# jyjblrd/Low-Cost-Mocap

Hardware: AMD Instinct MI355X
Metric: triangulated 3D markers/sec at 8 cams x 16 markers (higher is better)
Workload: dtype f64

## Files before the change

low-cost-mocap_amd/csrc/frame_bb.hip:

```cpp
#include "mocap_device.hpp"
#include "kernels.hpp"
#include <cstdlib>
#include "frame_common.hpp"
#include "bb_fold.hpp"

namespace mocap {

constexpr int kBBThreads = 256;
constexpr int kBBWaves = kBBThreads / 64;
constexpr int kBBRecs = kBBThreads + 64;
constexpr int bb_cw(int C) { return C <= 8 ? 1 : 2; }
constexpr uint32_t bb_rec_bytes(int CW) { return 24u + 8u * (uint32_t)CW; }
constexpr bool bb_group_rows(int CT, int ML, int RL) { return CT > 0 && ML > 0 && RL > 0 && CT * ML < 0xFF && (ML & (ML - 1)) == 0; }

constexpr int bb_wg_per_cu(int RL) { return RL == 48 ? 5 : 4; }
constexpr size_t kBBCacheEntry = 4;
constexpr int kBBLdsSlack = 1024;
struct BBLayout {
  size_t bxy, bxy_nx, cnt_nx, bt, rbound, seedkey, slot_key, claimw, recs, rpk, scr, scr_bytes, goff, gcnt, outslot, boff, bnb, seedgh, slot_g, cnt,
      misc, bpl, nh, hits, act, root_blob, root_cam, nact, bnl, bv, pkbase, seen, bcache, total;
  int ncache;
  __host__ __device__ static size_t al(size_t x, size_t a) { return (x + a - 1) / a * a; }
  __host__ __device__ BBLayout(int C, int M, int R, int CW, int wg_per_cu) {
    size_t o = 0;
    auto take = [&](size_t bytes, size_t a) {
      o = al(o, a);
      const size_t at = o;
      o += bytes;
      return at;
    };
    bxy = take(sizeof(float2) * (size_t)C * M, 16);
    bxy_nx = take(sizeof(float2) * (size_t)C * M, 16);
    cnt_nx = take(4 * (size_t)C, 4);
    bt = take(sizeof(double) * 10 * ((size_t)C * M + 1), 16);
    rbound = take(8 * (size_t)R, 8);
    claimw = take(8 * (size_t)C, 8);
    pkbase = take(8 * (size_t)CW * R, 8);
    scr = seedkey = take(8 * (size_t)R, 8);
    slot_key = take(8 * (size_t)kBBWaves * R, 8);
    recs = take(8 * (size_t)kBBRecs, 8);
    rpk = take(8 * (size_t)kBBRecs * CW, 8);
    seedgh = take(4 * (size_t)R, 4);
    slot_g = take(4 * (size_t)kBBWaves * R, 4);
    scr_bytes = o - scr;
    goff = take(4 * (size_t)(R + 1), 4);
    gcnt = take(4 * (size_t)R, 4);
    outslot = take(4 * (size_t)R, 4);
    boff = take(4 * (size_t)(R + 1), 4);
    bnb = take(4 * (size_t)R, 4);
    cnt = take(4 * (size_t)C, 4);
    misc = take(4 * 16, 4);
    bpl = take(2 * (size_t)R, 2);
    seen = take(2 * (size_t)R, 2);
    nh = take((size_t)R * C, 1);
    hits = take((size_t)R * C * M, 1);
    act = take((size_t)R * C, 1);
    root_blob = take((size_t)R, 1);
    root_cam = take((size_t)R, 1);
    nact = take((size_t)R, 1);
    bnl = take((size_t)R, 1);
    bv = take((size_t)R, 1);
    bcache = take(0, 4);
    ncache = 0;
    const size_t per_entry = kBBCacheEntry;
    for (int per_cu = wg_per_cu; per_cu >= 1; per_cu--) {
      const size_t lim = ((size_t)160 * 1024 / per_cu - kBBLdsSlack) / 256 * 256;
      if (lim >= o + per_entry * 64) {
        const size_t n = (lim - o) / per_entry;
        ncache = (int)(n > 1024 ? 1024 : n);
        break;
      }
    }
    o += per_entry * (size_t)ncache;
    total = al(o, 16);
  }
};

static int bb_fixed_slots(int C, int M, int R) {
  const char* e = getenv("MOCAP_BB_FIXED_LAYOUT");
  if (e && e[0] == '0') return 0;
  if (C == 8 && M == 16 && R <= 48) return 48;
  if (C == 8 && M == 16 && R <= 64) return 64;
  return 0;
}
static int frame_bb_root_slots(int C, int M, int R) {
  const int f = bb_fixed_slots(C, M, R);
  return f ? f : R;
}
size_t frame_bb_lds_bytes(int C, int M, int R) { return BBLayout(C, M, frame_bb_root_slots(C, M, R), bb_cw(C), bb_wg_per_cu(bb_fixed_slots(C, M, R))).total; }
static size_t frame_bb_lds_bytes_min(int C, int M, int R) {
  const BBLayout L(C, M, frame_bb_root_slots(C, M, R), bb_cw(C), bb_wg_per_cu(bb_fixed_slots(C, M, R)));
  return L.total - kBBCacheEntry * (size_t)L.ncache;
}
bool frame_bb_fits(int C, int M, int R) {
  return C >= 2 && C <= 16 && M >= 1 && M <= 64 && R >= 1 && R <= 255 && frame_bb_lds_bytes_min(C, M, R) <= (size_t)128 * 1024;
}

template <int CW, uint32_t NONE = 0xFFu>
struct Packed {
  unsigned long long w[CW];
  __device__ __forceinline__ void clear() {
#pragma unroll
    for (int k = 0; k < CW; k++) w[k] = NONE * 0x0101010101010101ull;
  }
  __device__ __forceinline__ void set(int c, uint32_t idx) {
    if (CW == 1)
      w[0] ^= (unsigned long long)(idx ^ NONE) << (8 * c);
    else
      w[c >> 3] ^= (unsigned long long)(idx ^ NONE) << (8 * (c & 7));
  }
  __device__ __forceinline__ uint32_t get(int c) const {
    return CW == 1 ? (uint32_t)(w[0] >> (8 * c)) & 0xFFu : (uint32_t)(w[c >> 3] >> (8 * (c & 7))) & 0xFFu;
  }
};

template <int CT, bool PERK = false>
struct BBCamTables {
  const double* base;
  static constexpr int C = CT;
  static constexpr int kPq = PERK ? 12 * CT * CT : 12 * CT;
  __device__ __forceinline__ ctab_t pq(size_t off) const { return as_ctab(base + off); }
  __device__ __forceinline__ ctab_t rt(size_t off) const { return as_ctab(base + kPq + off); }
  __device__ __forceinline__ ctab_t k4(size_t off) const { return as_ctab(base + kPq + 12 * CT + off); }
  __device__ __forceinline__ const double* f() const { return base + kPq + 16 * CT; }
};
template <bool PERK>
struct BBCamTables<0, PERK> {
  const double* base;
  int C;
  __device__ __forceinline__ ctab_t pq(size_t off) const { return as_ctab(base + off); }
  __device__ __forceinline__ ctab_t rt(size_t off) const { return as_ctab(base + (PERK ? 12 * C * C : 12 * C) + off); }
  __device__ __forceinline__ ctab_t k4(size_t off) const { return as_ctab(base + (PERK ? 12 * C * C + 12 * C : 24 * C) + off); }
  __device__ __forceinline__ const double* f() const { return base + (PERK ? 12 * C * C + 16 * C : 28 * C); }
};

enum { kPrioEval = 0, kPrioSeed = 1, kPrioPhase = 2, kPrioSerial = 3 };
template <int P>
__device__ __forceinline__ void bb_prio() {
  __builtin_amdgcn_s_setprio(P);
}

template <bool F32R, int CW, int CT, int ML, int RL, bool PERK = false>
struct BBState {
  static constexpr int T = kBBThreads, W = kBBWaves;
  static constexpr bool ROWS = bb_group_rows(CT, ML, RL);
  static constexpr uint32_t kNone = ROWS ? (uint32_t)(CT * ML) : 0xFFu;
  typedef Packed<CW, kNone> Pk;
  static constexpr bool PLIST = CT > 0 && ML > 0 && RL > 0 && ML < 32 && CT * ML <= 256 && (ML & (ML - 1)) == 0;
  __device__ __forceinline__ uint32_t gbyte(int c, uint32_t k) const { return ROWS ? (uint32_t)c * (uint32_t)ML + k : k; }
  __device__ __forceinline__ size_t grow(int c, uint32_t b) const { return ROWS ? (size_t)b : (size_t)c * M + b; }
  const FrameArgs& p;
  BBCamTables<CT, PERK> cv;
  const int C_, M, R, RS;
  int tid, lane, wave;
  __device__ __forceinline__ void fresh_tid() {
    int t = tid;
    asm volatile("" : "+v"(t));
    tid = t;
    lane = t & 63;
    wave = t >> 6;
  }
  __device__ __forceinline__ int cn() const { return CT > 0 ? CT : C_; }
  enum { PC_OTHER = 0, PC_PAIRS0, PC_PAIRS1, PC_B1_TABLE, PC_ROW_COPY, PC_PHASE_C, PC_SEED_PASS, PC_SEED_PUSH, PC_EVAL, PC_TEST, PC_PHASE_E, PC_COUNT };
#ifdef MOCAP_BB_PHASE_CLOCKS
  uint32_t pc_last = 0, pc_sum[PC_COUNT] = {};
  template <int PH>
  __device__ __forceinline__ void pc_mark() {
    if (__builtin_amdgcn_readfirstlane((int)threadIdx.x >> 6) == 0) {
      const uint32_t now = (uint32_t)__builtin_readcyclecounter();
      pc_sum[PH] += now - pc_last;
      pc_last = now;
    }
  }
  __device__ __forceinline__ void pc_start() { pc_last = (uint32_t)__builtin_readcyclecounter(); }
  __device__ __forceinline__ void pc_flush() const {
    if (threadIdx.x == 0 && !p.n_frames_dev)
      for (int k = 0; k < PC_COUNT; k++) atomicAdd(&p.status[p.n_frames + k], (int)(pc_sum[k] >> 8));
  }
#else
  template <int PH>
  __device__ __forceinline__ void pc_mark() {}
  __device__ __forceinline__ void pc_start() {}
  __device__ __forceinline__ void pc_flush() const {}
#endif
  double* bt;
  float2 *bxy, *bxy_nx;
  int32_t* cnt_nx;
  unsigned long long *rbound, *seedkey, *slot_key, *claimw, *rpk;
  struct BRec { uint32_t gh, rs; };
  BRec* recs;
  uint32_t *goff, *gcnt, *boff, *bnb, *seedgh, *slot_g;
  int32_t *outslot, *cnt, *misc;
  uint16_t* bpl;
  uint8_t *nh, *hits, *act, *root_blob, *root_cam, *nact, *bnl, *bv;
  float* bcache;
  unsigned long long* pkbase;
  uint16_t* seen;
  int ncache;
  unsigned char* scr;
  size_t scr_bytes;
  static constexpr unsigned long long kInfBits = 0x7ff0000000000000ull;

  __device__ BBState(const FrameArgs& p_, unsigned char* smem)
      : p(p_), C_(p_.cv.C), M(ML > 0 ? ML : p_.M), R(p_.K_max), RS(RL > 0 ? RL : p_.K_max), tid(threadIdx.x), lane(threadIdx.x & 63), wave(threadIdx.x >> 6) {
    const int C = cn();
    {
      const unsigned long long ta = (unsigned long long)(uintptr_t)p_.cv.Pq;
      uint32_t tlo = (uint32_t)__builtin_amdgcn_readfirstlane((int)(uint32_t)ta);
      uint32_t thi = (uint32_t)__builtin_amdgcn_readfirstlane((int)(uint32_t)(ta >> 32));
      asm volatile("" : "+s"(tlo), "+s"(thi));
      cv.base = (const double*)(uintptr_t)(((unsigned long long)thi << 32) | tlo);
      if constexpr (CT == 0) cv.C = C;
    }
    const BBLayout L(C, M, RS, CW, bb_wg_per_cu(RL));
    bt = (double*)(smem + L.bt);
    bxy = (float2*)(smem + L.bxy);
    bxy_nx = (float2*)(smem + L.bxy_nx);
    cnt_nx = (int32_t*)(smem + L.cnt_nx);
    rbound = (unsigned long long*)(smem + L.rbound);
    seedkey = (unsigned long long*)(smem + L.seedkey);
    slot_key = (unsigned long long*)(smem + L.slot_key);
    claimw = (unsigned long long*)(smem + L.claimw);
    recs = (BRec*)(smem + L.recs);
    rpk = (unsigned long long*)(smem + L.rpk);
    goff = (uint32_t*)(smem + L.goff);
    gcnt = (uint32_t*)(smem + L.gcnt);
    outslot = (int32_t*)(smem + L.outslot);
    boff = (uint32_t*)(smem + L.boff);
    bnb = (uint32_t*)(smem + L.bnb);
    seedgh = (uint32_t*)(smem + L.seedgh);
    slot_g = (uint32_t*)(smem + L.slot_g);
    cnt = (int32_t*)(smem + L.cnt);
    misc = (int32_t*)(smem + L.misc);
    bpl = (uint16_t*)(smem + L.bpl);
    nh = (uint8_t*)(smem + L.nh);
    hits = (uint8_t*)(smem + L.hits);
    act = (uint8_t*)(smem + L.act);
    root_blob = (uint8_t*)(smem + L.root_blob);
    root_cam = (uint8_t*)(smem + L.root_cam);
    nact = (uint8_t*)(smem + L.nact);
    bnl = (uint8_t*)(smem + L.bnl);
    bv = (uint8_t*)(smem + L.bv);
    scr = smem + L.scr;
    scr_bytes = L.scr_bytes;
    bcache = (float*)(smem + L.bcache);
    pkbase = (unsigned long long*)(smem + L.pkbase);
    seen = (uint16_t*)(smem + L.seen);
    ncache = L.ncache;
  }

  struct Line { double a, b, c, den, rden; };
  __device__ __forceinline__ Line epiline(int r, int i) const { return epiline_of(root_cam[r], root_blob[r], i); }
  __device__ __forceinline__ Line epiline_of(int rc, int rb, int i) const {
    const int C = cn();
    const double* Fm = cv.f() + 9 * ((size_t)rc * C + i);
    const float2 rp = bxy[(size_t)rc * M + rb];
    const double x = (double)rp.x, y = (double)rp.y;
    double a = Fm[0] * x + Fm[1] * y + Fm[2];
    double b = Fm[3] * x + Fm[4] * y + Fm[5];
    double c = Fm[6] * x + Fm[7] * y + Fm[8];
    double nu = a * a + b * b;
    nu = nu != 0.0 ? 1.0 / sqrt(nu) : 1.0;
    a *= nu;
    b *= nu;
    c *= nu;
    if (F32R) {
      a = (double)(float)a;
      b = (double)(float)b;
      c = (double)(float)c;
    }
    Line L;
    L.a = a;
    L.b = b;
    L.c = c;
    L.den = sqrt(a * a + b * b);
    L.rden = recip_refined(L.den);
    return L;
  }

  template <bool CHAIN>
  __device__ __forceinline__ unsigned long long match_pairs(const Line& mine, int pair_r, int pair_i, int n_pairs, int gs_shift,
                                                            int cam = 0, int Mi_chain = 0) {
    const int C = cn();
    const int GS = 1 << gs_shift, PPS = 64 >> gs_shift;
    const int k = lane & (GS - 1), q = lane >> gs_shift;
    const int gl0 = lane & ~(GS - 1);
    const unsigned long long gall = gs_shift == 6 ? ~0ull : ((1ull << GS) - 1ull);
    unsigned long long claims = 0ull;
    for (int s0 = 0; s0 < n_pairs; s0 += PPS) {
      const int src = s0 + q;
      const bool has = src < n_pairs;
      const int sl = has ? src : 0;
      const double la = __shfl(mine.a, sl), lb = __shfl(mine.b, sl), lc = __shfl(mine.c, sl);
      const double lden = __shfl(mine.den, sl), lrden = __shfl(mine.rden, sl);
      const int r = __shfl(pair_r, sl);
      const int i = CHAIN ? cam : __shfl(pair_i, sl);
      const int Mi = has ? (CHAIN ? Mi_chain : cnt[i]) : 0;
      const bool valid = k < Mi;
      float2 pt = make_float2(0.f, 0.f);
      double d = 0.0;
      bool hit = false;
      if (valid) {
        pt = bxy[(size_t)i * M + k];
        const double num = fabs(la * (double)pt.x + lb * (double)pt.y + lc);
        d = div_by(num, lden, lrden);
        hit = d < p.gate_px;
      }
      const unsigned long long wm = __ballot(hit);
      const unsigned long long gm = (wm >> gl0) & gall;
      int rank = 0;
      const unsigned int dlo = (unsigned int)__double_as_longlong(d), dhi = (unsigned int)(__double_as_longlong(d) >> 32);
      for (unsigned long long mm = wm; mm;) {
        const int j = __ffsll((long long)mm) - 1;
        mm &= mm - 1;
        const double dj = __longlong_as_double(((long long)__builtin_amdgcn_readlane((int)dhi, j) << 32) |
                                               (unsigned int)__builtin_amdgcn_readlane((int)dlo, j));
        const bool mine_grp = (j & ~(GS - 1)) == gl0 && j != lane;
        rank += (hit && mine_grp && (dj < d || (dj == d && j < lane))) ? 1 : 0;
      }
      if (hit) hits[((size_t)r * C + i) * M + rank] = (uint8_t)gbyte(i, (uint32_t)k);
      const unsigned long long g0 = (__ballot(hit && rank == 0) >> gl0) & gall;
      bool same = false;
      if (valid && g0) {
        const float2 p0 = bxy[(size_t)i * M + (__ffsll((long long)g0) - 1)];
        same = pt.x == p0.x && pt.y == p0.y;
      }
      const unsigned long long cw = __ballot(same);
      if (CHAIN) {
        for (int sh = 0; sh < 64; sh += GS) claims |= (cw >> sh) & gall;
      }
      if (has && k == 0) {
        nh[(size_t)r * C + i] = (uint8_t)__popcll(gm);
        if (!CHAIN) {
          const unsigned long long cm = (cw >> gl0) & gall;
          if (cm) atomicOr(&claimw[i], cm);
        }
      }
    }
    return claims;
  }

  __device__ __forceinline__ void prefetch_lds(int64_t frame) const {
    const int C = cn();
    const float* src = p.blobs + (size_t)frame * C * M * 2;
    const int n_dw = C * M * 2;
    for (int base = wave * 64; base < n_dw; base += T)
      if (base + lane < n_dw)
        __builtin_amdgcn_global_load_lds((const __attribute__((address_space(1))) void*)(src + base + lane),
                                         (__attribute__((address_space(3))) void*)((float*)bxy_nx + base), 4, 0, 0);
    if (wave == 0 && lane < C)
      __builtin_amdgcn_global_load_lds((const __attribute__((address_space(1))) void*)(p.counts + (size_t)frame * C + lane),
                                       (__attribute__((address_space(3))) void*)cnt_nx, 4, 0, 0);
  }
  __device__ __forceinline__ void stage(int64_t frame) {
    fresh_tid();
    const int C = cn();
    float2* t = bxy;
    bxy = bxy_nx;
    bxy_nx = t;
    if (tid < C) {
      const int n = cnt_nx[tid];
      cnt[tid] = n < 0 ? 0 : (n > M ? M : n);
      claimw[tid] = 0ull;
    }
    if (tid == 0) {
      misc[MI_STATUS] = 0;
      misc[MI_OMAX] = 0;
    }
  }

  __device__ void match() {
    fresh_tid();
    const int C = cn();
    __syncthreads();
    int gs_shift = 0;
    while ((1 << gs_shift) < M) gs_shift++;
    const int n0 = cnt[0] < R ? cnt[0] : R;
    {
      for (int r = tid; r < n0; r += T) {
        root_cam[r] = 0;
        root_blob[r] = (uint8_t)r;
      }
      if (tid == 0 && cnt[0] > R) misc[MI_STATUS] |= MOCAP_ST_ROOT_OVERFLOW_;
    }
    __syncthreads();
    auto U_of = [&](int j) {
      const int n = cnt[j];
      return ~claimw[j] & (n >= 64 ? ~0ull : ((1ull << n) - 1ull));
    };
    int n_prov = 0, n_ppairs = 0;
    bool pre = false;
    uint8_t* nh_s = nullptr;
    uint8_t* hits_s = nullptr;
    unsigned long long* pclaim = (unsigned long long*)scr;
    uint8_t* plist = act;
    uint32_t* p_end = goff;
    {
      int Mmax = 0;
      for (int c = 1; c < C; c++) Mmax = cnt[c] > Mmax ? cnt[c] : Mmax;
#pragma nounroll
      for (int stage_ = 0; stage_ < 2; stage_++) {
        const int stage = __builtin_amdgcn_readfirstlane(stage_);
        int NP = n0 * (C - 1);
        if (stage == 1) {
          block_sync_lds();
          pc_mark<PC_PAIRS0>();
          if constexpr (PLIST) {
#pragma unroll
            for (int j = 1; j < CT; j++) {
              const uint32_t U = ~((const uint32_t*)claimw)[2 * j] & ((1u << cnt[j]) - 1u);
              if (lane < ML && ((U >> lane) & 1u)) plist[__builtin_amdgcn_mbcnt_lo(U, (uint32_t)n_prov)] = (uint8_t)(j * ML + lane);
              n_prov += __popc(U);
              n_ppairs += __popc(U) * (CT - 1 - j);
              if (lane == 0) p_end[j] = ((uint32_t)n_ppairs << 16) | (uint32_t)n_prov;
            }
            wave_lds_sync();
          } else
          for (int j = 1; j < C; j++) {
            const int np = __popcll(U_of(j));
            n_prov += np;
            n_ppairs += np * (C - 1 - j);
          }
          pre = n_prov <= 64 && (size_t)n_prov * C * (8 + 1 + (size_t)M) <= scr_bytes;
          if (!pre) break;
          nh_s = (uint8_t*)(pclaim + (size_t)n_prov * C);
          hits_s = nh_s + (size_t)n_prov * C;
          NP = n_ppairs;
        }
        for (int base = wave * 64; base < NP; base += W * 64) {
          const int pi = base + lane;
          const bool have = pi < NP;
          int r = 0, i = 1, Mi = 0;
          Line L = {0, 0, 0, 1, 1};
          if (have) {
            if (stage == 0) {
              r = pi / (C - 1);
              i = 1 + (pi - r * (C - 1));
              L = epiline(r, i);
            } else if constexpr (PLIST) {
              int j = 1;
              uint32_t before = 0;
              const uint32_t key = ((uint32_t)pi << 16) | 0xFFFFu;
              uint32_t pe[CT > 2 ? CT - 2 : 1];
#pragma unroll
              for (int jj = 1; jj <= CT - 2; jj++) pe[jj - 1] = p_end[jj];
#pragma unroll
              for (int jj = 1; jj <= CT - 2; jj++) {
                const bool ge = key >= pe[jj - 1];
                j += ge ? 1 : 0;
                before = ge ? pe[jj - 1] : before;
              }
              const uint32_t acc = before >> 16, pb = before & 0xFFFFu;
              uint32_t ord, off;
              divmod_tiny((uint32_t)pi - acc, (uint32_t)(CT - 1 - j), ord, off);
              r = (int)(pb + ord);
              const int k = plist[r] & (ML - 1);
              i = j + 1 + (int)off;
              L = epiline_of(j, k, i);
            } else {
              int j = 1, acc = 0, pb = 0, span = C - 2;
              unsigned long long U = 0ull;
              for (; j <= C - 2; j++) {
                span = C - 1 - j;
                U = U_of(j);
                const int nj = __popcll(U) * span;
                if (pi < acc + nj) break;
                acc += nj;
                pb += __popcll(U);
              }
              uint32_t ord, off;
              divmod_tiny((uint32_t)(pi - acc), (uint32_t)span, ord, off);
              for (uint32_t t = 0; t < ord; t++) U &= U - 1;
              const int k = __ffsll((long long)U) - 1;
              i = j + 1 + (int)off;
              r = pb + (int)ord;
              L = epiline_of(j, k, i);
            }
            Mi = cnt[i];
          }
          const float2* pts = bxy + (size_t)i * M;
          auto dist = [&](int k) {
            const float2 pt = pts[k];
            return div_by(fabs(L.a * (double)pt.x + L.b * (double)pt.y + L.c), L.den, L.rden);
          };
          unsigned long long hm = 0ull;
#pragma unroll 4
          for (int k = 0; k < Mmax; k++)
            if (k < Mi && dist(k) < p.gate_px) hm |= 1ull << k;
          uint8_t* nhp = stage == 0 ? nh : nh_s;
          uint8_t* hl = (stage == 0 ? hits : hits_s) + ((size_t)r * C + i) * M;
          if (have) nhp[(size_t)r * C + i] = (uint8_t)__popcll(hm);
          unsigned long long rem = hm, claim = 0ull;
          int pos = 0;
          float2 p0 = make_float2(0.f, 0.f);
          while (__ballot(rem != 0ull)) {
            if (rem) {
              double bd = __builtin_huge_val();
              int bk = 0;
              for (unsigned long long t = rem; t; t &= t - 1) {
                const int k = __ffsll((long long)t) - 1;
                const double d = dist(k);
                if (d < bd) {
                  bd = d;
                  bk = k;
                }
              }
              hl[pos] = (uint8_t)gbyte(i, (uint32_t)bk);
              if (pos == 0) {
                p0 = pts[bk];
                for (unsigned long long t = hm; t; t &= t - 1) {
                  const int k = __ffsll((long long)t) - 1;
                  const float2 q = pts[k];
                  if (q.x == p0.x && q.y == p0.y) claim |= 1ull << k;
                }
              }
              rem &= ~(1ull << bk);
              pos++;
            }
          }
          if (stage == 0) {
            if (claim) atomicOr(&claimw[i], claim);
          } else if (have) {
            pclaim[(size_t)r * C + i] = claim;
          }
        }
      }
    }
    const int NL = M * ((C - 1) * (C - 2) / 2);
    const bool spec = F32R && (size_t)NL * 20 + 8 <= scr_bytes;
    double* sp_den = (double*)scr;
    float* sp_abc = (float*)(sp_den + NL);
    auto sp_base = [&](int j) { return M * ((j - 1) * (C - 1) - (j - 1) * j / 2); };
    if (spec && !pre) {
      int tot = 0;
      for (int j = 1; j <= C - 2; j++) {
        const int n = cnt[j];
        const unsigned long long U = ~claimw[j] & (n >= 64 ? ~0ull : ((1ull << n) - 1ull));
        tot += __popcll(U) * (C - 1 - j);
      }
      for (int l = tid; l < tot; l += T) {
        int j = 1, acc = 0, span = C - 2;
        unsigned long long U = 0ull;
        for (; j <= C - 2; j++) {
          const int n = cnt[j];
          U = ~claimw[j] & (n >= 64 ? ~0ull : ((1ull << n) - 1ull));
          span = C - 1 - j;
          const int nj = __popcll(U) * span;
          if (l < acc + nj) break;
          acc += nj;
        }
        uint32_t ord, off;
        divmod_tiny((uint32_t)(l - acc), (uint32_t)span, ord, off);
        for (uint32_t t = 0; t < ord; t++) U &= U - 1;
        const int k = __ffsll((long long)U) - 1, i = j + 1 + (int)off;
        const int ll = sp_base(j) + k * span + (int)off;
        const Line L = epiline_of(j, k, i);
        sp_den[ll] = L.den;
        sp_abc[3 * ll + 0] = (float)L.a;
        sp_abc[3 * ll + 1] = (float)L.b;
        sp_abc[3 * ll + 2] = (float)L.c;
      }
    }
    __syncthreads();
    pc_mark<PC_PAIRS1>();
    fresh_tid();
    if (wave == 0) bb_prio<kPrioSerial>();
    if (wave == 0 && pre) {
      int jp = 0, kp = 0;
      if constexpr (PLIST) {
        if (lane < n_prov) {
          const int row = plist[lane];
          jp = row / ML;
          kp = row & (ML - 1);
        }
      } else
      if (lane < n_prov) {
        int acc = 0;
        unsigned long long U = 0ull;
        for (jp = 1; jp < C; jp++) {
          U = U_of(jp);
          const int np = __popcll(U);
          if (lane < acc + np) break;
          acc += np;
        }
        for (int t = 0; t < lane - acc; t++) U &= U - 1;
        kp = __ffsll((long long)U) - 1;
      }
      bool real = false;
      for (int i = 1; i < C; i++) {
        wave_lds_sync();
        if (lane < n_prov && jp == i) {
          real = !((claimw[i] >> kp) & 1ull);
          if (real)
            for (int c = i + 1; c < C; c++) {
              const unsigned long long m = pclaim[(size_t)lane * C + c];
              if (m) atomicOr(&claimw[c], m);
            }
        }
      }
      const unsigned long long rm = __ballot(real);
      const int rank = __popcll(rm & ((1ull << lane) - 1ull));
      int n_roots = n0 + __popcll(rm);
      if (real && n0 + rank < R) {
        root_cam[n0 + rank] = (uint8_t)jp;
        root_blob[n0 + rank] = (uint8_t)kp;
        bnl[rank] = (uint8_t)lane;
      }
      if (lane == 0) {
        if (n_roots > R) {
          misc[MI_STATUS] |= MOCAP_ST_ROOT_OVERFLOW_;
          n_roots = R;
        }
        misc[MI_NROOTS] = n_roots;
      }
    } else if (wave == 0) {
      const int cntL = lane < C ? cnt[lane] : 0;
      const unsigned long long clmL = lane < C ? claimw[lane] : 0ull;
      int nr_cam = 0, nr_blob = 0;
      int n_roots = n0;
      bool over = false;
      for (int i = 1; i < C; i++) {
        const int Mi = __builtin_amdgcn_readlane(cntL, i);
        unsigned long long claimed = ((unsigned long long)(unsigned int)__builtin_amdgcn_readlane((int)(clmL >> 32), i) << 32) |
                                     (unsigned int)__builtin_amdgcn_readlane((int)clmL, i);
        const int n_new = n_roots - n0;
        for (int base = 0; base < n_new; base += 64) {
          const int l = base + lane;
          const bool have = l < n_new;
          int j = nr_cam, k = nr_blob;
          if (base) {
            wave_lds_sync();
            j = have ? root_cam[n0 + l] : 0;
            k = have ? root_blob[n0 + l] : 0;
          }
          Line L = {0, 0, 0, 1, 1};
          if (have) {
            if (spec) {
              const int ll = sp_base(j) + k * (C - 1 - j) + (i - j - 1);
              L.a = (double)sp_abc[3 * ll + 0];
              L.b = (double)sp_abc[3 * ll + 1];
              L.c = (double)sp_abc[3 * ll + 2];
              L.den = sp_den[ll];
              L.rden = recip_refined(L.den);
            } else {
              L = epiline_of(j, k, i);
            }
          }
          claimed |= match_pairs<true>(L, n0 + l, i, (n_new - base < 64) ? n_new - base : 64, gs_shift, i, Mi);
        }
        const bool flag = lane < Mi && !((claimed >> lane) & 1ull);
        const unsigned long long mask = __ballot(flag);
        const int pos = __popcll(mask & ((1ull << lane) - 1ull));
        if (flag) {
          const int rr = n_roots + pos;
          if (rr < R) {
            root_cam[rr] = (uint8_t)i;
            root_blob[rr] = (uint8_t)lane;
          }
        }
        int slot = n_new;
        for (unsigned long long mm = mask; mm; slot++) {
          const int jb = __ffsll((long long)mm) - 1;
          mm &= mm - 1;
          if (lane == slot) {
            nr_cam = i;
            nr_blob = jb;
          }
        }
        n_roots += __popcll(mask);
        if (n_roots > R) {
          over = true;
          n_roots = R;
        }
      }
      if (lane == 0) {
        if (over) misc[MI_STATUS] |= MOCAP_ST_ROOT_OVERFLOW_;
        misc[MI_NROOTS] = n_roots;
      }
    } else {
      float om = 0.0f;
      for (int i = tid - 64; i < C * M; i += T - 64) {
        const int c = i / M, k = i - c * M;
        if (k < cnt[c]) {
          const float2 v = bxy[i];
          om = fmaxf(om, fmaxf(fabsf(v.x), fabsf(v.y)));
          double Bc[10];
          dlt_contribution(Bc, cv.pq(PERK ? 12 * (c * C + c) : 12 * c), (double)v.x, (double)v.y);
#pragma unroll
          for (int e = 0; e < 10; e++) bt[(size_t)i * 10 + e] = Bc[e];
        }
      }
      if (om > 0.0f) atomicMax(&misc[MI_OMAX], __float_as_int(om));
      if (tid == 64) {
        const int it = q_add(&p.q.counters[QC_NEXT_FRAME], 1);
        misc[MI_NEXT] = it < frame_count(p) ? it : -1;
      }
    }
    bb_prio<kPrioPhase>();
    __syncthreads();
    pc_mark<PC_B1_TABLE>();
    if (pre) {
      const int n_new = misc[MI_NROOTS] - n0;
      for (int idx = tid; idx < n_new * C; idx += T) {
        const int q = idx / C, c = idx - q * C;
        const int r = n0 + q, ps = bnl[q];
        if (c > (int)root_cam[r]) {
          const int n = nh_s[(size_t)ps * C + c];
          nh[(size_t)r * C + c] = (uint8_t)n;
          const uint8_t* src = hits_s + ((size_t)ps * C + c) * M;
          uint8_t* dst = hits + ((size_t)r * C + c) * M;
          for (int t = 0; t < n; t++) dst[t] = src[t];
        }
      }
      __syncthreads();
      pc_mark<PC_ROW_COPY>();
    }

    fresh_tid();
    const int nroots = misc[MI_NROOTS];
    for (int r = tid; r < nroots; r += T) {
      const int rc = root_cam[r];
      unsigned long long total = 1;
      int views = 1, na = 0;
      bool over = false;
      Pk pkb;
      pkb.clear();
      pkb.set(rc, gbyte(rc, root_blob[r]));
      uint32_t sm = 1u << rc;
      for (int c = rc + 1; c < C; c++) {
        const unsigned n = nh[(size_t)r * C + c];
        if (n > 1) act[(size_t)r * C + na++] = (uint8_t)c;
        if (n == 1) pkb.set(c, hits[((size_t)r * C + c) * M]);
        if (n) {
          sm |= 1u << c;
          views++;
          total *= n;
          if (total > (unsigned long long)p.G_cap) {
            over = true;
            total = 1;
          }
        }
      }
      if (over) atomicOr(&misc[MI_STATUS], MOCAP_ST_CAND_OVERFLOW_);
      nact[r] = (uint8_t)na;
      bv[r] = (uint8_t)views;
#pragma unroll
      for (int k = 0; k < CW; k++) pkbase[(size_t)r * CW + k] = pkb.w[k];
      if (PERK) seen[r] = (uint16_t)sm;
      rbound[r] = kInfBits;
      const uint32_t g = (views > 1 && !over) ? (uint32_t)total : 0u;
      gcnt[r] = g;
      {
        const uint8_t* a = act + (size_t)r * C;
        uint32_t pl = 1, nb = 1;
        int nl = 0;
        for (int k = 0; k < na; k++) nb *= nh[(size_t)r * C + a[k]];
        if (over) nb = 1;
        while (nl < na && (pl < (uint32_t)p.bb_pl_min || (pl < (uint32_t)p.bb_pl && nb > (uint32_t)p.bb_nb_max))) {
          const uint32_t n = nh[(size_t)r * C + a[nl++]];
          uint32_t dummy;
          pl *= n;
          divmod_small(nb, n, nb, dummy);
        }
        bpl[r] = (uint16_t)pl;
        bnl[r] = (uint8_t)nl;
        bnb[r] = g ? nb : 0u;
        seedkey[r] = 0ull;
        seedgh[r] = 0xFFFFFFFFu;
      }
    }
    for (int s = tid; s < W * RS; s += T) {
      slot_key[s] = ~0ull;
      slot_g[s] = 0xFFFFFFFFu;
    }
    if (tid == 0) misc[MI_BBCTR] = misc[MI_BBCTR2] = 0;
    __syncthreads();
    if (wave == 0) bb_prio<kPrioSerial>();
    if (wave == 0) {
      uint32_t carry = 0, bcarry = 0;
      int slots = 0;
      for (int base = 0; base < nroots; base += 64) {
        const int r = base + lane;
        const uint32_t g = r < nroots ? gcnt[r] : 0u;
        const uint32_t nb = r < nroots ? bnb[r] : 0u;
        const uint32_t incl = wave_inclusive_scan(g, lane);
        const uint32_t bincl = wave_inclusive_scan(nb, lane);
        const unsigned long long nz = __ballot(g != 0u);
        if (r < nroots) {
          goff[r] = carry + incl - g;
          boff[r] = bcarry + bincl - nb;
          outslot[r] = g ? slots + __popcll(nz & ((1ull << lane) - 1ull)) : -1;
        }
        carry += (uint32_t)__builtin_amdgcn_readlane((int)incl, 63);
        bcarry += (uint32_t)__builtin_amdgcn_readlane((int)bincl, 63);
        slots += __popcll(nz);
      }
      if (lane == 0) {
        goff[nroots] = carry;
        boff[nroots] = bcarry;
        misc[MI_NOUT] = slots;
        misc[MI_G] = misc[MI_STATUS] ? 0 : (int32_t)carry;
      }
    }
    bb_prio<kPrioPhase>();
    __syncthreads();
    pc_mark<PC_PHASE_C>();
  }

  __device__ __forceinline__ void add_view(double (&B)[10], int c, uint32_t k, int j) const {
    if (PERK && j != c) {
      const float2 w = bxy[grow(c, k)];
      double Bc[10];
      dlt_contribution(Bc, cv.base + 12 * ((size_t)j * cn() + c), (double)w.x, (double)w.y);
#pragma unroll
      for (int e = 0; e < 10; e++) B[e] = B[e] + Bc[e];
    } else {
      const double* t = bt + grow(c, k) * 10;
#pragma unroll
      for (int e = 0; e < 10; e++) B[e] = B[e] + t[e];
    }
  }

  template <bool WITH_B>
  __device__ __forceinline__ int group_matrix(int r, uint32_t rem, int skip, double (&B)[10], Pk& pk) const {
    const int C = cn();
    const int rc = root_cam[r];
    const uint8_t* nhr = nh + (size_t)r * C;
    const uint8_t* hr = hits + (size_t)r * C * M;
    pk.clear();
    int v = 0, ka = 0;
    int j = 0;
    if (WITH_B) {
#pragma unroll
      for (int e = 0; e < 10; e++) B[e] = 0.0;
    }
    for (int c = 0; c < C; c++) {
      uint32_t k = kNone;
      bool seen = false;
      if (c == rc) {
        k = gbyte(c, root_blob[r]);
        seen = true;
      } else if (c > rc) {
        const uint32_t n = nhr[c];
        seen = n != 0;
        if (n == 1) {
          k = hr[(size_t)c * M];
        } else if (n > 1) {
          if (ka >= skip) {
            uint32_t qd, dgt;
            if (rem < 8192u) divmod_tiny(rem, n, qd, dgt); else
            divmod_small(rem, n, qd, dgt);
            rem = qd;
            k = hr[(size_t)c * M + dgt];
          }
          ka++;
        }
      }
      if (k != kNone) {
        if (WITH_B) add_view(B, c, k, j);
        v++;
        pk.set(c, k);
      }
      if (PERK) j += seen ? 1 : 0;
    }
    return v;
  }

  __device__ __forceinline__ void block_pk(int r, uint32_t gh, Pk& pk) const {
    const int C = cn();
#pragma unroll
    for (int k = 0; k < CW; k++) pk.w[k] = pkbase[(size_t)r * CW + k];
    const uint8_t* a = act + (size_t)r * C;
    const int na = nact[r];
    uint32_t rem = gh;
    for (int k = bnl[r]; k < na; k++) {
      const int c = a[k];
      const uint32_t n = nh[(size_t)r * C + c];
      uint32_t qd, dgt;
      if (rem < 8192u) divmod_tiny(rem, n, qd, dgt); else
      divmod_small(rem, n, qd, dgt);
      rem = qd;
      pk.set(c, hits[((size_t)r * C + c) * M + dgt]);
    }
  }
  __device__ __forceinline__ int block_matrix(int r, uint32_t gh, Pk& pk, double (&B)[10]) const {
    const int C = cn();
    block_pk(r, gh, pk);
#pragma unroll
    for (int ee = 0; ee < 10; ee++) B[ee] = 0.0;
    if constexpr (PERK) {
      const uint32_t sm = seen[r];
#pragma unroll CT > 0 ? CT : 1
      for (int c = 0; c < C; c++) {
        const uint32_t k = pk.get(c);
        if (k != kNone) add_view(B, c, k, __popc(sm & ((1u << c) - 1u)));
      }
    } else {
#pragma unroll CT > 0 ? CT : 1
      for (int c = 0; c < C; c++) {
        const uint32_t k = pk.get(c);
        const double* t = bt + (size_t)(ROWS ? k : k != 0xFFu ? (uint32_t)c * (uint32_t)M + k : (uint32_t)C * (uint32_t)M) * 10;
#pragma unroll
        for (int ee = 0; ee < 10; ee++) B[ee] = B[ee] + t[ee];
      }
    }
    return (int)bv[r] - (int)bnl[r];
  }

  __device__ __forceinline__ int fetch_candidate(uint32_t lo, uint32_t i, int& r, uint32_t& gl, Pk& pk, double (&B)[10]) const {
    const int C = cn();
    const BRec rec = recs[lo];
    r = (int)(rec.rs & 0xFFu);
#pragma unroll
    for (int k = 0; k < CW; k++) pk.w[k] = rpk[(size_t)lo * CW + k];
    if (rec.rs >> 31) {
      gl = rec.gh;
    } else {
      uint32_t rem = i - (rec.rs >> 8);
      gl = rec.gh * (uint32_t)bpl[r] + rem;
      const uint8_t* a = act + (size_t)r * C;
      const int nl = bnl[r];
      for (int k = 0; k < nl; k++) {
        const int c = a[k];
        uint32_t qd, dgt;
        divmod_tiny(rem, nh[(size_t)r * C + c], qd, dgt);
        rem = qd;
        pk.set(c, hits[((size_t)r * C + c) * M + dgt]);
      }
    }
#pragma unroll
    for (int ee = 0; ee < 10; ee++) B[ee] = 0.0;
    if constexpr (PERK) {
      int j = 0;
#pragma unroll CT > 0 ? CT : 1
      for (int c = 0; c < C; c++) {
        const uint32_t k = pk.get(c);
        if (k != kNone) add_view(B, c, k, j++);
      }
    } else {
#pragma unroll CT > 0 ? CT : 1
      for (int c = 0; c < C; c++) {
        const uint32_t k = pk.get(c);
        const double* t = bt + (size_t)(ROWS ? k : k != 0xFFu ? (uint32_t)c * (uint32_t)M + k : (uint32_t)C * (uint32_t)M) * 10;
#pragma unroll
        for (int ee = 0; ee < 10; ee++) B[ee] = B[ee] + t[ee];
      }
    }
    return bv[r];
  }

  __device__ void search(bool bound_tests) {
    fresh_tid();
    const int C = cn();
    (void)C;
    __builtin_amdgcn_s_waitcnt(0x0F70);
    const int nroots = misc[MI_NROOTS];
    int32_t* ctr = &misc[MI_BBCTR];
    int32_t* ctr_other = &misc[MI_BBCTR2];
    const double inf = __builtin_huge_val();
    EigCut ec;
    {
      const double om = (double)__int_as_float(misc[MI_OMAX]);
      ec.p3max2 = p.p3max2;
      ec.o2slack = (1100.0 * 0x1p-46) * (om * om);
    }
    const double c0[3] = {p.bb_c0[0], p.bb_c0[1], p.bb_c0[2]};
    const uint32_t nblocks = boff[nroots];
    auto root_of_block = [&](uint32_t b_first_of_wave, uint32_t b) {
      return coop_last_le([&](int r) { return boff[r]; }, nroots, b_first_of_wave, b, lane);
    };
    auto push_block = [&](int r, uint32_t gh, const Pk& pk) {
      const uint32_t old = (uint32_t)atomicAdd(ctr, (int32_t)(((uint32_t)bpl[r] << 10) | 1u));
      const uint32_t slot = old & 0x3FFu;
      BRec rec;
      rec.gh = gh;
      rec.rs = (uint32_t)r | ((old >> 10) << 8);
      recs[slot] = rec;
#pragma unroll
      for (int k = 0; k < CW; k++) rpk[(size_t)slot * CW + k] = pk.w[k];
    };
    auto rec_start = [&](int k) { return (recs[k].rs & 0x7FFFFFFFu) >> 8; };
    auto root_y = [&](int r) {
      const int vf = bv[r];
      const double bound = __longlong_as_double((long long)rbound[r]);
      const double limit = bound * (double)(2 * vf) * (1.0 + 0x1p-40);
      const double limit_adj = fma(1.002, limit, (double)(2 * vf) * ec.o2slack);
      return p.p3max2c * limit_adj;
    };
    auto dropped = [&](int r, double s1, double tr) { return s1 * fma(2e-12, tr, root_y(r)) < 1.0; };
    if (bound_tests) {
      bb_prio<kPrioSeed>();
      int my_r = -1;
      uint32_t my_gh = 0;
      unsigned long long my_key = 0ull;
      Pk my_pk;
      my_pk.clear();
      for (uint32_t s0 = 0; s0 < nblocks; s0 += T) {
        const uint32_t b = s0 + (uint32_t)tid;
        if (s0 + (uint32_t)(wave * 64) >= nblocks) continue;
        const int r = root_of_block(s0 + (uint32_t)(wave * 64), b < nblocks ? b : nblocks - 1);
        if (b < nblocks) {
          const uint32_t gh = b - boff[r];
          double B[10], tr = 0.0;
          Pk pk;
          const int v = block_matrix(r, gh, pk, B);
          double s1d = __builtin_huge_val();
          float s1 = 0.0f;
          if (v >= 2) {
            s1d = eigcut_s1_shifted(B, c0, tr);
            s1 = (float)fmin(s1d, 3e38);
          }
          if (b < (uint32_t)ncache) bcache[b] = v >= 2 ? bb_fold_bound(s1d, tr) : bb_fold_inf();
          my_key = ((unsigned long long)__float_as_uint(s1) << 32) | (unsigned long long)(0xFFFFFFFFu - gh);
          my_r = r;
          my_gh = gh;
          my_pk = pk;
          atomicMax(&seedkey[r], my_key);
        }
      }
      block_sync_lds_only();
      pc_mark<PC_SEED_PASS>();
      if (nblocks <= (uint32_t)T) {
        if (my_r >= 0 && seedkey[my_r] == my_key) {
          seedgh[my_r] = my_gh;
          push_block(my_r, my_gh, my_pk);
        }
      } else
      for (int r = tid; r < nroots; r += T) {
        if (bnb[r]) {
          const uint32_t gh = 0xFFFFFFFFu - (uint32_t)seedkey[r];
          seedgh[r] = gh;
          seedkey[r] = 0ull;
          Pk pk;
          block_pk(r, gh, pk);
          push_block(r, gh, pk);
        }
      }
      bb_prio<kPrioEval>();
      block_sync_lds_only();
      pc_mark<PC_SEED_PUSH>();
    }
    uint32_t b0 = 0;
    fresh_tid();
    while (true) {
      const uint32_t cv_ = (uint32_t)*ctr;
      const uint32_t ns = cv_ & 0x3FFu, ne = cv_ >> 10;
      const bool blocks_left = b0 < nblocks;
      const bool full = ns > (uint32_t)(kBBRecs - T);
      if (ns && (full || !blocks_left || ne >= (uint32_t)p.bb_flush)) {
        for (uint32_t i0 = 0; i0 < ne; i0 += T) {
          const uint32_t i = i0 + (uint32_t)tid;
          const bool have = i < ne;
          double e = inf, X[3] = {0, 0, 0};
          int r = 0;
          uint32_t gl = 0;
          uint32_t lo = 0;
          if (i0 + (uint32_t)(wave * 64) < ne)
            lo = (uint32_t)coop_last_le(rec_start, (int)ns, i0 + (uint32_t)(wave * 64), have ? i : ne - 1, lane);
          Pk pk;
          pk.clear();
          if (have) {
            double B[10];
            const int v = fetch_candidate(lo, i, r, gl, pk, B);
            if constexpr (ROWS) {
#pragma unroll
              for (int k = 0; k < CW; k++) asm volatile("" : "+v"(pk.w[k]));
            }
            auto obs_p = [&](int c, double& x, double& y) -> bool {
              const uint32_t k = pk.get(c);
              if (k == kNone) return false;
              const float2 w = bxy[grow(c, k)];
              x = (double)w.x;
              y = (double)w.y;
              return true;
            };
            const double bound = __longlong_as_double((long long)rbound[r]);
            solve_and_score<!PERK, true, F32R, false, 1, true>(cv, B, v, obs_p, X, e, bound * (double)(2 * v) * (1.0 + 0x1p-40), ec);
#ifdef MOCAP_DEBUG_EIGCHECK
            if (!(e < inf)) {
              double B2[10], X2[3], e2;
#pragma unroll
              for (int ee = 0; ee < 10; ee++) B2[ee] = 0.0;
              int j2 = 0;
              for (int c = 0; c < C; c++) {
                const uint32_t k = pk.get(c);
                if (k != kNone) add_view(B2, c, k, j2++);
              }
              solve_and_score<!PERK, true, F32R>(cv, B2, v, obs_p, X2, e2);
              atomicAdd(&p.status[p.n_frames], 1);
              if (e2 <= bound) printf("EIGCHECK candidate: root %d g %u bound %.17g true %.17g\n", r, gl, bound, e2);
            }
#endif
          }
          const bool fin = e < inf;
          const unsigned long long key = fin ? (unsigned long long)__double_as_longlong(e) : kInfBits;
          const uint32_t gword = (gl << 1) | ((e != e) ? 1u : 0u);
          const int ss = wave * RS + r;
          if (fin) atomicMin(&rbound[r], key);
          const bool want = have && (key < slot_key[ss] || (key == slot_key[ss] && gword < slot_g[ss]));
          if (__ballot(want)) {
            unsigned long long old = 0;
            if (want) old = atomicMin(&slot_key[ss], key);
            wave_lds_sync();
            const bool holder = want && slot_key[ss] == key;
            if (holder && old > key) slot_g[ss] = 0xFFFFFFFFu;
            wave_lds_sync();
            if (holder) atomicMin(&slot_g[ss], gword);
            wave_lds_sync();
            if (holder && slot_g[ss] == gword) store_winner(ss, X, pk);
          }
        }
        block_sync_lds_only();
        pc_mark<PC_EVAL>();
        if (tid == 0) *ctr = 0;
        {
          int32_t* t = ctr;
          ctr = ctr_other;
          ctr_other = t;
        }
        continue;
      }
      if (!blocks_left) break;
      const uint32_t b = b0 + (uint32_t)tid;
      const uint32_t bw = b0 + (uint32_t)(wave * 64);
      b0 += T;
      int r = 0;
      if (bw < nblocks) r = root_of_block(bw, b < nblocks ? b : nblocks - 1);
      bool do_push = false;
      uint32_t gh = 0;
      Pk pk;
      pk.clear();
      if (b < nblocks) {
        gh = b - boff[r];
        if (gh != seedgh[r]) {
          double B[10], tr;
          bool survive = true;
          if (bound_tests && b < (uint32_t)ncache) {
            survive = !bb_fold_dropped(bcache[b], root_y(r));
            if (survive) block_pk(r, gh, pk);
          } else if (bound_tests) {
            const int v = block_matrix(r, gh, pk, B);
            if (v >= 2) {
              const double s1 = eigcut_s1_shifted(B, c0, tr);
              survive = !dropped(r, s1, tr);
            }
          } else {
            block_pk(r, gh, pk);
          }
          do_push = survive;
#ifdef MOCAP_DEBUG_EIGCHECK
          if (!survive) {
            const double bound = __longlong_as_double((long long)rbound[r]);
            const uint32_t pl = bpl[r];
            for (uint32_t l = 0; l < pl; l++) {
              double B2[10], X2[3], e2 = inf;
              Pk pk2;
              const int v2 = group_matrix<true>(r, gh * pl + l, 0, B2, pk2);
              auto obs2 = [&](int c, double& x, double& y) -> bool {
                const uint32_t k = pk2.get(c);
                if (k == kNone) return false;
                const float2 w = bxy[grow(c, k)];
                x = (double)w.x;
                y = (double)w.y;
                return true;
              };
              solve_and_score<!PERK, true, F32R>(cv, B2, v2, obs2, X2, e2);
              atomicAdd(&p.status[p.n_frames + 1], 1);
              if (e2 <= bound) printf("EIGCHECK block: root %d block %u candidate %u bound %.17g true %.17g\n", r, gh, l, bound, e2);
            }
          }
#endif
        }
      }
      block_sync_lds_only();
      if (do_push) push_block(r, gh, pk);
      block_sync_lds_only();
      pc_mark<PC_TEST>();
    }
    wait_own_stores();
    __syncthreads();
  }

  __device__ __forceinline__ bool root_winner(int r, unsigned long long& kb, uint32_t& gw, int& wb) const {
    kb = ~0ull;
    gw = 0xFFFFFFFFu;
    wb = 0;
    for (int w = 0; w < W; w++) {
      const int s = w * RS + r;
      const unsigned long long k = slot_key[s];
      const uint32_t g = slot_g[s];
      if (k < kb || (k == kb && g < gw)) {
        kb = k;
        gw = g;
        wb = w;
      }
    }
    return kb != ~0ull;
  }

  static constexpr uint32_t kRecBytes = bb_rec_bytes(CW);
  __device__ __forceinline__ unsigned char* winner_rec(int s) const {
    return p.ws + (size_t)blockIdx.x * p.ws_stride + (size_t)(kRecBytes * (uint32_t)s);
  }
  __device__ __forceinline__ void store_winner(int s, const double (&X)[3], const Pk& pk) const {
    unsigned long long* rec = (unsigned long long*)winner_rec(s);
    if constexpr (CW == 1) {
      typedef unsigned long long rec2_t __attribute__((ext_vector_type(2)));
      const rec2_t lo = {(unsigned long long)__double_as_longlong(X[0]), (unsigned long long)__double_as_longlong(X[1])};
      const rec2_t hi = {(unsigned long long)__double_as_longlong(X[2]), pk.w[0]};
      ((rec2_t*)rec)[0] = lo;
      ((rec2_t*)rec)[1] = hi;
    } else {
#pragma unroll
      for (int k = 0; k < 3; k++) rec[k] = (unsigned long long)__double_as_longlong(X[k]);
#pragma unroll
      for (int k = 0; k < CW; k++) rec[3 + k] = pk.w[k];
    }
  }
  __device__ static __forceinline__ uint32_t row_word(uint32_t two) {
    const uint32_t x = (two & 0xFFu) | ((two & 0xFF00u) << 8);
    if constexpr (ROWS) {
      static_assert(!ROWS || kNone == 0x80u, "row_word: the record of zeros is the byte with bit 7 set");
      return (x & ((uint32_t)(ML - 1) * 0x00010001u)) | ((x >> 7) & 0x00010001u) * 0xFFFFu;
    }
    const uint32_t none = ((x + 0x00010001u) >> 8) & 0x00010001u;
    return x | none * 0xFF00u;
  }
  __device__ void write_point(int64_t frame, int r) const {
    const int C = cn();
    unsigned long long kb;
    uint32_t gw;
    int wv;
    if (!root_winner(r, kb, gw, wv)) return;
    const double e = kb != kInfBits ? __longlong_as_double((long long)kb)
                                    : ((gw & 1u) ? __longlong_as_double(0x7ff8000000000000ll) : __builtin_huge_val());
    const size_t o = (size_t)frame * R + outslot[r];
    const unsigned long long* rec = (const unsigned long long*)winner_rec(wv * RS + r);
    unsigned long long w[3 + CW];
#pragma unroll
    for (int k = 0; k < 3 + CW; k++) w[k] = q_ld(rec + k);
    p.err[o] = e;
    const double X[3] = {__longlong_as_double((long long)w[0]), __longlong_as_double((long long)w[1]), __longlong_as_double((long long)w[2])};
    int16_t* co = p.corr + o * C;
    if constexpr (CT == 8) {
      typedef uint32_t row_t __attribute__((ext_vector_type(4), aligned(2)));
      const uint32_t lo = (uint32_t)w[3], hi = (uint32_t)(w[3] >> 32);
      row_t v = {row_word(lo), row_word(lo >> 16), row_word(hi), row_word(hi >> 16)};
      *(row_t*)co = v;
    } else {
      for (int c = 0; c < C; c++) {
        const uint32_t k = (uint32_t)(w[3 + (CW == 1 ? 0 : c >> 3)] >> (8 * (c & 7))) & 0xFFu;
        co[c] = k == kNone ? (int16_t)-1 : (int16_t)(ROWS ? k & (uint32_t)(ML - 1) : k);
      }
    }
    store_point(p, o, X);
  }
};

template <bool F32R, int CW, int CT, int ML, int RL>
__global__ __launch_bounds__(kBBThreads, bb_wg_per_cu(RL)) void frame_bb_kernel(FrameArgs p) {
  extern __shared__ __attribute__((aligned(16))) unsigned char smem[];
#define BB_STATE BBState<F32R, CW, CT, ML, RL>
#include "frame_bb_body.inc"
#undef BB_STATE
}

template <bool F32R, int CW, int CT, int ML, int RL>
__global__ __launch_bounds__(kBBThreads, bb_wg_per_cu(RL)) void frame_bb_calib_kernel(FrameArgs p) {
  extern __shared__ __attribute__((aligned(16))) unsigned char smem[];
#define BB_STATE BBState<F32R, CW, CT, ML, RL, true>
#include "frame_bb_body.inc"
#undef BB_STATE
}

int frame_bb_wg_per_cu_cap(int C, int M, int R) { return bb_wg_per_cu(bb_fixed_slots(C, M, R)); }
size_t frame_bb_ws_bytes(int) { return BBLayout::al(bb_rec_bytes(2) * (size_t)kBBWaves * 255, 256); }
static_assert(bb_wg_per_cu(48) <= kBBMaxWgPerCu && bb_wg_per_cu(64) <= kBBMaxWgPerCu && bb_wg_per_cu(0) <= kBBMaxWgPerCu, "frame_capi.hip sizes the workspace for kBBMaxWgPerCu workgroups per CU");

hipError_t launch_frame_bb(const FrameArgs& a, int grid, hipStream_t stream) {
  const size_t lds = frame_bb_lds_bytes(a.cv.C, a.M, a.K_max);
  if (!a.ws || a.ws_stride < bb_rec_bytes(bb_cw(a.cv.C)) * (size_t)kBBWaves * (size_t)frame_bb_root_slots(a.cv.C, a.M, a.K_max)) return hipErrorInvalidValue;
  const size_t nPq = a.cv.uniformK ? (size_t)12 * a.cv.C : (size_t)12 * a.cv.C * a.cv.C;
  if (a.cv.RT != a.cv.Pq + nPq || a.cv.K4 != a.cv.RT + 12 * a.cv.C || a.cv.F != a.cv.K4 + 4 * a.cv.C) return hipErrorInvalidValue;
  void (*k)(FrameArgs);
  const bool f32 = a.cv.f32_rounding != 0;
  const int fixed = bb_fixed_slots(a.cv.C, a.M, a.K_max);
  if (fixed && fixed != 48 && fixed != 64) return hipErrorInvalidValue;
  static_assert(bb_cw(8) == 1 && bb_cw(9) == 2 && bb_cw(16) == 2, "BB_PICK takes CW = 1 up to eight cameras, CW = 2 above");
#define BB_PICK(KERNEL)                                                                             \
  (fixed == 48       ? (f32 ? KERNEL<true, 1, 8, 16, 48> : KERNEL<false, 1, 8, 16, 48>)             \
   : fixed == 64     ? (f32 ? KERNEL<true, 1, 8, 16, 64> : KERNEL<false, 1, 8, 16, 64>)             \
   : a.cv.C == 8     ? (f32 ? KERNEL<true, 1, 8, 0, 0> : KERNEL<false, 1, 8, 0, 0>)                 \
   : a.cv.C <= 8     ? (f32 ? KERNEL<true, 1, 0, 0, 0> : KERNEL<false, 1, 0, 0, 0>)                 \
                     : (f32 ? KERNEL<true, 2, 0, 0, 0> : KERNEL<false, 2, 0, 0, 0>))
  k = a.cv.uniformK ? BB_PICK(frame_bb_kernel) : BB_PICK(frame_bb_calib_kernel);
#undef BB_PICK
  if (lds > 48 * 1024) {
    hipError_t e = hipFuncSetAttribute((const void*)k, hipFuncAttributeMaxDynamicSharedMemorySize, (int)lds);
    if (e != hipSuccess) return e;
  }
  hipLaunchKernelGGL(k, dim3(grid), dim3(kBBThreads), lds, stream, a);
  return hipGetLastError();
}

}
```

Baseline: 624.1 million.

## Pack per-root nh/act rows into 64-bit words and track nearest hit during gating

```diff
diff --git a/low-cost-mocap_amd/csrc/frame_bb.hip b/low-cost-mocap_amd/csrc/frame_bb.hip
--- a/low-cost-mocap_amd/csrc/frame_bb.hip
+++ b/low-cost-mocap_amd/csrc/frame_bb.hip
@@ -21,7 +21,7 @@
       misc, bpl, nh, hits, act, root_blob, root_cam, nact, bnl, bv, pkbase, seen, bcache, total;
   int ncache;
   __host__ __device__ static size_t al(size_t x, size_t a) { return (x + a - 1) / a * a; }
-  __host__ __device__ BBLayout(int C, int M, int R, int CW, int wg_per_cu) {
+  __host__ __device__ BBLayout(int C, int M, int R, int CW, int wg_per_cu, bool row_words = false) {
     size_t o = 0;
     auto take = [&](size_t bytes, size_t a) {
       o = al(o, a);
@@ -52,9 +52,9 @@
     misc = take(4 * 16, 4);
     bpl = take(2 * (size_t)R, 2);
     seen = take(2 * (size_t)R, 2);
-    nh = take((size_t)R * C, 1);
+    nh = take((size_t)R * C, row_words ? 8 : 1);
     hits = take((size_t)R * C * M, 1);
-    act = take((size_t)R * C, 1);
+    act = take((size_t)R * C, row_words ? 8 : 1);
     root_blob = take((size_t)R, 1);
     root_cam = take((size_t)R, 1);
     nact = take((size_t)R, 1);
@@ -87,9 +87,9 @@
   const int f = bb_fixed_slots(C, M, R);
   return f ? f : R;
 }
-size_t frame_bb_lds_bytes(int C, int M, int R) { return BBLayout(C, M, frame_bb_root_slots(C, M, R), bb_cw(C), bb_wg_per_cu(bb_fixed_slots(C, M, R))).total; }
+size_t frame_bb_lds_bytes(int C, int M, int R) { return BBLayout(C, M, frame_bb_root_slots(C, M, R), bb_cw(C), bb_wg_per_cu(bb_fixed_slots(C, M, R)), bb_fixed_slots(C, M, R) != 0).total; }
 static size_t frame_bb_lds_bytes_min(int C, int M, int R) {
-  const BBLayout L(C, M, frame_bb_root_slots(C, M, R), bb_cw(C), bb_wg_per_cu(bb_fixed_slots(C, M, R)));
+  const BBLayout L(C, M, frame_bb_root_slots(C, M, R), bb_cw(C), bb_wg_per_cu(bb_fixed_slots(C, M, R)), bb_fixed_slots(C, M, R) != 0);
   return L.total - kBBCacheEntry * (size_t)L.ncache;
 }
 bool frame_bb_fits(int C, int M, int R) {
@@ -146,6 +146,9 @@
   static constexpr bool ROWS = bb_group_rows(CT, ML, RL);
   static constexpr uint32_t kNone = ROWS ? (uint32_t)(CT * ML) : 0xFFu;
   typedef Packed<CW, kNone> Pk;
+  static_assert(!ROWS || (CT == 8 && CW == 1), "a row of nh / act as one word: eight cameras");
+  __device__ __forceinline__ unsigned long long row_word64(const uint8_t* rows, int r) const { return ((const unsigned long long*)rows)[r]; }
+  __device__ static __forceinline__ uint32_t byte_of(unsigned long long w, uint32_t k) { return (uint32_t)(w >> (8u * k)) & 0xFFu; }
   static constexpr bool PLIST = CT > 0 && ML > 0 && RL > 0 && ML < 32 && CT * ML <= 256 && (ML & (ML - 1)) == 0;
   __device__ __forceinline__ uint32_t gbyte(int c, uint32_t k) const { return ROWS ? (uint32_t)c * (uint32_t)ML + k : k; }
   __device__ __forceinline__ size_t grow(int c, uint32_t b) const { return ROWS ? (size_t)b : (size_t)c * M + b; }
@@ -212,7 +215,7 @@
       cv.base = (const double*)(uintptr_t)(((unsigned long long)thi << 32) | tlo);
       if constexpr (CT == 0) cv.C = C;
     }
-    const BBLayout L(C, M, RS, CW, bb_wg_per_cu(RL));
+    const BBLayout L(C, M, RS, CW, bb_wg_per_cu(RL), ROWS);
     bt = (double*)(smem + L.bt);
     bxy = (float2*)(smem + L.bxy);
     bxy_nx = (float2*)(smem + L.bxy_nx);
@@ -484,6 +487,22 @@
             return div_by(fabs(L.a * (double)pt.x + L.b * (double)pt.y + L.c), L.den, L.rden);
           };
           unsigned long long hm = 0ull;
+          double bd0 = __builtin_huge_val();
+          int bk0 = 0;
+          if constexpr (ROWS) {
+#pragma unroll 4
+            for (int k = 0; k < Mmax; k++)
+              if (k < Mi) {
+                const double d = dist(k);
+                if (d < p.gate_px) {
+                  hm |= 1ull << k;
+                  if (d < bd0) {
+                    bd0 = d;
+                    bk0 = k;
+                  }
+                }
+              }
+          } else
 #pragma unroll 4
           for (int k = 0; k < Mmax; k++)
             if (k < Mi && dist(k) < p.gate_px) hm |= 1ull << k;
@@ -493,10 +512,30 @@
           unsigned long long rem = hm, claim = 0ull;
           int pos = 0;
           float2 p0 = make_float2(0.f, 0.f);
+          if constexpr (ROWS) {
+            if (hm) {
+              hl[0] = (uint8_t)gbyte(i, (uint32_t)bk0);
+              claim = hm;
+              if (hm & (hm - 1ull)) {
+                claim = 0ull;
+                p0 = pts[bk0];
+                for (unsigned long long t = hm; t; t &= t - 1) {
+                  const int k = __ffsll((long long)t) - 1;
+                  const float2 q = pts[k];
+                  if (q.x == p0.x && q.y == p0.y) claim |= 1ull << k;
+                }
+              }
+              rem = hm & ~(1ull << bk0);
+              pos = 1;
+            }
+          }
           while (__ballot(rem != 0ull)) {
             if (rem) {
               double bd = __builtin_huge_val();
               int bk = 0;
+              if (ROWS && !(rem & (rem - 1ull))) {
+                bk = __ffsll((long long)rem) - 1;
+              } else
               for (unsigned long long t = rem; t; t &= t - 1) {
                 const int k = __ffsll((long long)t) - 1;
                 const double d = dist(k);
@@ -506,7 +545,7 @@
                 }
               }
               hl[pos] = (uint8_t)gbyte(i, (uint32_t)bk);
-              if (pos == 0) {
+              if (!ROWS && pos == 0) {
                 p0 = pts[bk];
                 for (unsigned long long t = hm; t; t &= t - 1) {
                   const int k = __ffsll((long long)t) - 1;
@@ -719,6 +758,61 @@
     fresh_tid();
     const int nroots = misc[MI_NROOTS];
     for (int r = tid; r < nroots; r += T) {
+      if constexpr (ROWS) {
+        const uint32_t rc = root_cam[r], rb = root_blob[r];
+        unsigned long long nw = row_word64(nh, r);
+        const uint8_t* hr = hits + (size_t)r * (CT * ML);
+        uint32_t h1[CT];
+#pragma unroll
+        for (int c = 1; c < CT; c++) h1[c] = hr[c * ML];
+        nw &= (~0ull << (8u * rc)) << 8;
+        Pk pkb;
+        pkb.clear();
+        pkb.set((int)rc, gbyte((int)rc, rb));
+        static_assert(CT <= 8 && ML <= 16, "a digit's byte: three bits of camera, four of hit count - 1");
+        unsigned long long ew = 0ull;
+        uint32_t total = 1, views = 1, na = 0, sm = 1u << rc;
+#pragma unroll
+        for (int c = CT - 1; c >= 1; c--) {
+          const uint32_t n = byte_of(nw, (uint32_t)c);
+          if (n > 1) {
+            ew = (ew << 8) | (unsigned long long)((n << 3) + (uint32_t)(c - 8));
+            na++;
+          }
+          if (n == 1) pkb.set(c, h1[c]);
+          if (n) {
+            sm |= 1u << c;
+            views++;
+            total *= n;
+          }
+        }
+        const unsigned long long aw = ew & 0x0707070707070707ull;
+        const unsigned long long dn = ((ew >> 3) & 0x0F0F0F0F0F0F0F0Full) + 0x0101010101010101ull;
+        const bool over = (unsigned long long)total > (unsigned long long)p.G_cap;
+        if (over) atomicOr(&misc[MI_STATUS], MOCAP_ST_CAND_OVERFLOW_);
+        ((unsigned long long*)act)[r] = aw;
+        nact[r] = (uint8_t)na;
+        bv[r] = (uint8_t)views;
+        pkbase[r] = pkb.w[0];
+        if (PERK) seen[r] = (uint16_t)sm;
+        rbound[r] = kInfBits;
+        const uint32_t g = (views > 1 && !over) ? total : 0u;
+        gcnt[r] = g;
+        uint32_t pl = 1, nb = over ? 1u : total;
+        uint32_t nl = 0;
+        while (nl < na && (pl < (uint32_t)p.bb_pl_min || (pl < (uint32_t)p.bb_pl && nb > (uint32_t)p.bb_nb_max))) {
+          const uint32_t n = byte_of(dn, nl++);
+          uint32_t dummy;
+          pl *= n;
+          divmod_small(nb, n, nb, dummy);
+        }
+        bpl[r] = (uint16_t)pl;
+        bnl[r] = (uint8_t)nl;
+        bnb[r] = g ? nb : 0u;
+        seedkey[r] = 0ull;
+        seedgh[r] = 0xFFFFFFFFu;
+        continue;
+      }
       const int rc = root_cam[r];
       unsigned long long total = 1;
       int views = 1, na = 0;
@@ -870,6 +964,21 @@
     const int C = cn();
 #pragma unroll
     for (int k = 0; k < CW; k++) pk.w[k] = pkbase[(size_t)r * CW + k];
+    if constexpr (ROWS) {
+      const unsigned long long aw = row_word64(act, r), nw = row_word64(nh, r);
+      const int na = nact[r];
+      const uint8_t* hr = hits + (size_t)r * (CT * ML);
+      uint32_t rem = gh;
+      for (int k = bnl[r]; k < na; k++) {
+        const uint32_t c = byte_of(aw, (uint32_t)k), n = byte_of(nw, c);
+        uint32_t qd, dgt;
+        if (rem < 8192u) divmod_tiny(rem, n, qd, dgt); else
+        divmod_small(rem, n, qd, dgt);
+        rem = qd;
+        pk.set((int)c, hr[c * (uint32_t)ML + dgt]);
+      }
+      return;
+    }
     const uint8_t* a = act + (size_t)r * C;
     const int na = nact[r];
     uint32_t rem = gh;
@@ -920,6 +1029,17 @@
       gl = rec.gh * (uint32_t)bpl[r] + rem;
       const uint8_t* a = act + (size_t)r * C;
       const int nl = bnl[r];
+      if constexpr (ROWS) {
+        const unsigned long long aw = row_word64(act, r), nw = row_word64(nh, r);
+        const uint8_t* hr = hits + (size_t)r * (CT * ML);
+        for (int k = 0; k < nl; k++) {
+          const uint32_t c = byte_of(aw, (uint32_t)k);
+          uint32_t qd, dgt;
+          divmod_tiny(rem, byte_of(nw, c), qd, dgt);
+          rem = qd;
+          pk.set((int)c, hr[c * (uint32_t)ML + dgt]);
+        }
+      } else
       for (int k = 0; k < nl; k++) {
         const int c = a[k];
         uint32_t qd, dgt;
```

After: 647.3 million (median of 6 runs). 3.7% higher.
